# h3poteto/aws-global-accelerator-controller

Hardware: NVIDIA H100
Metric: objects reconciled/sec at 10^6 Service+Ingress; change-set bit-exact vs Go ref (higher is better)
Workload: dtype u8/u32 (bytes and indices)

## Files before the change

aws-global-accelerator-controller_b200/csrc/gar_common.h:

```cpp
#pragma once

#include <stdint.h>
#include <stddef.h>

#include "../../include/garecon.h"

#if defined(__CUDACC__)
#define GAR_HD __host__ __device__ __forceinline__
#define GAR_D __device__ __forceinline__
#else
#define GAR_HD inline
#define GAR_D inline
#endif

#if defined(__CUDA_ARCH__)
#define GAR_ANY(p) __any_sync(0xffffffffu, (p))
#else
bool gar_host_vote(bool p);
#define GAR_ANY(p) gar_host_vote((p))
#endif

typedef uint8_t u8;
typedef uint16_t u16;
typedef uint32_t u32;
// ... 238 lines not shown
  if (p.loaded) p.e = load_entry(ix.ent + p.c.pos);
  return p;
}
GAR_HD bool idx_next(const HashIdx &ix, PreCursor &p, IdxEntry *out) {
  while (p.c.pos < p.c.end) {
    if (!p.loaded) p.e = load_entry(ix.ent + p.c.pos);
    p.loaded = false;
    p.c.pos++;
    if (p.e.tag == p.c.tag) {
      *out = p.e;
      return true;
    }
  }
  return false;
}
```

aws-global-accelerator-controller_b200/csrc/gar_delta.h:

```cpp
#pragma once

#include <stddef.h>
#include <string.h>

#include <algorithm>
#include <string>
#include <unordered_map>
#include <unordered_set>
#include <vector>

#include "gar_pipeline.h"

enum DeltaCol {
  DC_KIND, DC_SPEC, DC_FLAGS, DC_NS, DC_NAME, DC_ICLS, DC_ANN_B, DC_LBI_B, DC_PORT_B, DC_ANN_KEY, DC_ANN_VAL, DC_LBI_HOST, DC_PORT_NUM,
  DC_PORT_PROTO, DC_N
};
enum ActualCol {
  AC_LB_REGION, AC_LB_NAME, AC_LB_DNS, AC_LB_ARN, AC_LB_STATE, AC_ACC_NAME, AC_ACC_DNS, AC_ACC_ENABLED, AC_ACC_TAG_B, AC_ACC_LIS_B, AC_TAG_KEY,
  AC_TAG_VAL, AC_LIS_PROTO, AC_LIS_PR_B, AC_LIS_EG_B, AC_PR_FROM, AC_EG_EP_B, AC_EP_ID, AC_ZONE_NAME, AC_ZONE_REC_B, AC_REC_NAME, AC_REC_TYPE,
  AC_REC_ALIAS, AC_REC_ALIAS_DNS, AC_REC_VAL_B, AC_VAL_VALUE, AC_N
};
enum ActualTable { AT_LB, AT_ACC, AT_TAG, AT_LIS, AT_PR, AT_EG, AT_EP, AT_ZONE, AT_REC, AT_VAL, AT_N };
enum DeltaScratch {
  DS_UP = 0, DS_KEY_KIND = DC_N, DS_KEY_REF, DS_KEY_SLAB, DS_COUNTS, DS_OFFS, DS_ROWS, DS_PAIRS, DS_SRC, DS_TOTALS,
  DS_A_UP, DS_A_SRC = DS_A_UP + AC_N, DS_A_DEL = DS_A_SRC + AT_N, DS_A_PAIRS = DS_A_DEL + AT_N, DS_A_ZTARGET = DS_A_PAIRS + AT_N, DS_A_ZREF,
  DS_A_ZSLAB, DS_A_FLAG, DS_A_COL, DS_N = DS_A_COL + 2 * AC_N
};

constexpr u32 SRC_UPSERT = 0x80000000u;

struct FDeltaResolve {
  DevTables T;
  HashIdx ix;
  const u8 *kind;
  const gar_str *key;
  const u8 *slab;
  u32 *counts;
  const u32 *offs;
  u32 *rows;
  GAR_HD void operator()(u32 k) const {
    const u32 kd = kind[k];
    const Str ks = mkstr(slab, key[k]);
    Cursor c = idx_open(ix, key_hash_kinded(kd, ks));
    IdxEntry e;
    u32 m = 0;
    while (idx_next(ix, c, &e))
      if (e.a0 == kd && streq(mkstr(T.o.slab, e.s0), ks)) {
        if (rows) rows[offs[k] + m] = e.row;
        m++;
      }
    if (!rows) counts[k] = m;
  }
};
struct FDeltaIdentity {
  u32 *src;
  GAR_HD void operator()(u32 i) const { src[i] = i; }
};
struct FDeltaScatter {
  const u32 *pairs;
  u32 *src;
  GAR_HD void operator()(u32 k) const { src[pairs[2 * k]] = pairs[2 * k + 1]; }
};
// ... 719 lines not shown
```

aws-global-accelerator-controller_b200/csrc/gar_pipeline.h:

```cpp
#pragma once

#include <stdio.h>
#include <stdlib.h>

#include <initializer_list>

#include "gar_rows.h"

#if defined(__CUDA_ARCH__)
#define GAR_ATOMIC_ADD(p, v) atomicAdd((p), (v))
#else
#define GAR_ATOMIC_ADD(p, v) (*(p) += (v))
#endif


enum Slot {
  S_DERIVED, S_OFLAGS, S_OKEY_HASH, S_STAGE_GA, S_STAGE_R53, S_ANN_R53, S_ANN_NAME, S_ANN_TAGS, S_ANN_LISTEN, S_DPORT_BEGIN, S_DPORTS,
  S_TOK_CODE, S_TOK_NAME, S_TOK_REGION,
  S_ACC_FLAGS, S_ACC_OWNER_KEY, S_ACC_OWNER, S_ACC_THOST, S_ACC_MANAGED, S_ACC_OWNER_HASH, S_ACC_THOST_HASH, S_REC_NAME_HASH, S_VAL_KEY_HASH,
  S_REC_ZONE, S_VAL_REC, S_VAL_CLS, S_VAL_KEY, S_VAL_ORPHAN, S_VAL_LINK, S_ACC_DIGEST,
  S_R53_MODE, S_R53_ACC, S_R53_ACC_DNS, S_PAIR_BEGIN, S_PAIR_OBJ, S_PAIR_HN, S_PAIR_CODE, S_PAIR_ZONE, S_PAIR_REC,
  S_IX_LB, S_IX_OWNER = S_IX_LB + 3, S_IX_THOST = S_IX_OWNER + 3, S_IX_ZONE = S_IX_THOST + 3, S_IX_VAL = S_IX_ZONE + 3,
  S_IX_ALIAS = S_IX_VAL + 3, S_IX_OBJ = S_IX_ALIAS + 3, S_IX_OVN = S_IX_OBJ + 3,
  S_SORT_KEYS = S_IX_OVN + 3, S_SORT_VALS, S_SORT_KEYS_ALT, S_SORT_VALS_ALT, S_SORT_TAGS,
  S_COUNTS, S_STATUS_GA, S_STATUS_R53, S_OPS, S_ERRFLAG, S_IX_EG, S_IX_EG_ENT, S_IX_EG_PAD,
  S_VAL_OBJ, S_ACC_OBJ, S_OBJ_CANON, S_OWN_BEGIN, S_OWN_FILL, S_OWN_ENT, S_OWN_MULTI,
  S_IXA_BEGIN, S_IXA_FILL, S_IXA_ENT, S_IXA_MULTI, S_OVN_FILL, S_OVN_MULTI, S_LB_HASH, S_REC_FLAGS, S_LBI_RES,
  S_NSLOTS
};


struct FClassify {
  DevTables T;
  Work W;
  u32 *derived_public;
  u8 *oflags;
  u32 *errflag;
  GAR_HD void operator()(u32 i) const {
    classify_object(T, W, i);
    W.obj_canon[i] = i;
    u32 dv = W.derived[i];
    if (dv & OBJ_KEY_BAD) GAR_ATOMIC_ADD(errflag, 1u);
// ... 130 lines not shown
    }
    W.dport_begin[i] = n;
  }
};
struct FJsonWrite {
  DevTables T;
  Work W;
  GAR_HD void operator()(u32 i) const {
    if (!(W.derived[i] & GAR_DV_PORTS_FROM_ANN)) return;
    if (W.dport_begin[i + 1] == W.dport_begin[i] || W.dport_begin[i + 1] > W.dport_cap) return;
    u32 stk[GAR_JSON_STACK_WORDS];
    json_listen_ports(mkstr(T.o.slab, W.ann_listen[i]), W.dports + W.dport_begin[i], stk);
  }
};

struct FLbHash {
  DevTables T;
  Work W;
  GAR_HD void operator()(u32 i) const {
    u64 h = key_hash_lb(mkstr(T.a.slab, T.a.lb_region[i]), mkstr(T.a.slab, T.a.lb_name[i]));
    W.lb_hash[i] = h;
    ix_count(W.hist[IX_LB], h);
  }
};
struct FRowLb {
  DevTables T;
  Work W;
  GAR_HD bool make(u32 i, u64 *h, IdxEntry *e) const {
    *h = W.lb_hash[i];
    e->a0 = T.a.lb_state[i];
    e->a1 = 0;
    e->s0 = T.a.lb_name[i];
    e->s1 = T.a.lb_region[i];
    return true;
  }
};
struct FRowOwner {
  DevTables T;
  Work W;
  GAR_HD bool make(u32 i, u64 *h, IdxEntry *e) const {
    u32 fl = W.acc_flags[i];
    *h = W.acc_owner_hash[i];
    e->a0 = fl;
    e->a1 = 0;
    e->s0 = W.acc_owner_key[i];
    e->s1 = 0;
    return (fl & ACC_MINE) && (fl & ACC_OWNER_KEYED) && i < W.acc_guest_from;
  }
// ... 57 lines not shown
struct FRowAlias {
  DevTables T;
  Work W;
  GAR_HD bool make(u32 r, u64 *h, IdxEntry *e) const {
    *h = key_hash_zoned_h(W.rec_zone[r], W.rec_name_hash[r]);
    e->a0 = W.rec_zone[r];
    e->a1 = T.a.rec_type[r];
    e->s0 = T.a.rec_name[r];
    e->s1 = T.a.rec_alias_dns[r];
    return T.a.rec_has_alias[r] != 0;
  }
};
struct FRowObj {
  DevTables T;
  Work W;
  GAR_HD bool make(u32 i, u64 *h, IdxEntry *e) const {
    gar_str ns = T.o.obj_ns[i];
    *h = W.okey_hash[i];
    e->a0 = T.o.obj_kind[i];
    e->a1 = 0;
    e->s0 = GAR_STR(GAR_STR_OFF(ns), GAR_STR_LEN(ns) + 1 + GAR_STR_LEN(T.o.obj_name[i]));
    e->s1 = 0;
    return !(W.derived[i] & OBJ_KEY_BAD);
  }
};
struct FRowOvn {
  DevTables T;
  Work W;
  GAR_HD bool make(u32 v, u64 *h, IdxEntry *e) const {
    u32 rec = W.val_rec[v];
    *h = key_hash_zoned_h(W.rec_zone[rec], W.rec_name_hash[rec]);
    e->a0 = rec;
    e->a1 = W.rec_zone[rec];
    e->s0 = T.a.rec_name[rec];
    e->s1 = T.a.val_value[v];
    return W.val_orphan[v] != 0;
  }
};

constexpr u32 IDX_SMALL_BUCKET = 48;
struct CanonHook {
  u32 *canon;
  const u8 *slab;
  u32 b0, b1;
  GAR_HD void operator()(u32 b, const IdxEntry *ent, u32 lo, u32 m) const {
    if (canon && b >= b0 && b < b1) canon_bucket(ent, lo, m, slab, canon);
  }
};
template <class RowF>
struct FIdxRows {
  RowF rowf;
  u32 *keys, *vals;
  IdxEntry *tmp;
  u32 *counts;
  u32 mask, nb;
  GAR_HD void operator()(u32 i) const {
    u64 h = 0;
    IdxEntry e;
    bool valid = rowf.make(i, &h, &e);
    u32 k = valid ? hash_bucket(h, mask) : nb;
    keys[i] = k;
    if (vals) vals[i] = i;
    if (valid) {
      e.tag = hash_tag(h);
      e.row = i;
      tmp[i] = e;
      GAR_ATOMIC_ADD(&counts[k], 1u);
    }
  }
};
struct FIdxPlace {
  const u32 *keys;
  u32 *cursor;
  const IdxEntry *tmp;
  IdxEntry *ent;
  u32 nb;
  GAR_HD void operator()(u32 i) const {
    u32 k = keys[i];
    if (k == nb) return;
#if defined(__CUDA_ARCH__)
    u32 pos = atomicAdd(&cursor[k], 1u);
#else
    u32 pos = cursor[k]++;
#endif
    ent[pos] = tmp[i];
  }
};
struct FIdxOrder {
  const u32 *begin;
  IdxEntry *ent;
  u32 *overflow;
  CanonHook canon;
  GAR_HD void operator()(u32 b) const {
    u32 lo = begin[b], m = begin[b + 1] - lo;
    if (m < 2) return;
    if (m > IDX_SMALL_BUCKET) {
      GAR_ATOMIC_ADD(overflow, 1u);
      return;
    }
    for (u32 k = 1; k < m; k++) {
      IdxEntry x = ent[lo + k];
      u32 j = k;
      while (j > 0 && ent[lo + j - 1].row > x.row) {
        ent[lo + j] = ent[lo + j - 1];
        j--;
      }
      if (j != k) ent[lo + j] = x;
    }
    canon(b, ent, lo, m);
  }
};
struct FIdxGather {
  const u32 *vals;
  const u32 *nvalid;
  const IdxEntry *tmp;
  IdxEntry *ent;
  GAR_HD void operator()(u32 p) const {
    if (p < *nvalid) ent[p] = tmp[vals[p]];
  }
};
struct FIdxCanon {
  const u32 *begin;
  const IdxEntry *ent;
  CanonHook canon;
  GAR_HD void operator()(u32 b) const {
    const u32 lo = begin[b], m = begin[b + 1] - lo;
    if (m >= 2) canon(b, ent, lo, m);
  }
};
template <class RowF>
struct FIdxPlaceDirect {
  RowF rowf;
  u32 *cursor;
  IdxEntry *ent;
  u32 mask;
  GAR_HD void operator()(u32 i) const {
    u64 h = 0;
    IdxEntry e;
    if (!rowf.make(i, &h, &e)) return;
    const u32 k = hash_bucket(h, mask);
#if defined(__CUDA_ARCH__)
    const u32 pos = atomicAdd(&cursor[k], 1u);
#else
    const u32 pos = cursor[k]++;
#endif
    e.tag = hash_tag(h);
    e.row = i;
    ent[pos] = e;
  }
};
struct FIdxMultiList {
  const u32 *begin;
  u32 *multi;
  GAR_HD void operator()(u32 b) const {
    const bool m = begin[b + 1] - begin[b] >= 2;
#if defined(__CUDA_ARCH__)
    const unsigned active = __activemask();
    const unsigned votes = __ballot_sync(active, m);
    if (!m) return;
    const unsigned lane = threadIdx.x & 31u;
    const int leader = __ffs(votes) - 1;
    u32 base = 0;
    if ((int)lane == leader) base = atomicAdd(multi, (u32)__popc(votes));
    base = __shfl_sync(votes, base, leader);
    multi[1 + base + __popc(votes & ((1u << lane) - 1u))] = b;
#else
    if (m) multi[1 + multi[0]++] = b;
#endif
  }
};
struct FIdxOrderMulti {
  const u32 *begin;
  IdxEntry *ent;
  const u32 *multi;
  u32 *overflow;
  CanonHook canon;
  GAR_HD void operator()(u32 t) const {
    const u32 b = multi[1 + t];
    const u32 lo = begin[b], m = begin[b + 1] - lo;
    if (m > IDX_SMALL_BUCKET) {
      GAR_ATOMIC_ADD(overflow, 1u);
      return;
    }
    for (u32 k = 1; k < m; k++) {
      IdxEntry x = ent[lo + k];
      u32 j = k;
      while (j > 0 && ent[lo + j - 1].row > x.row) {
        ent[lo + j] = ent[lo + j - 1];
        j--;
      }
      if (j != k) ent[lo + j] = x;
    }
    canon(b, ent, lo, m);
  }
};
enum FlagWord { FW_BAD_KEYS = 0, FW_IDX_OVERFLOW = 1, FW_NDPORTS = 2, FW_NPAIRS = 3, FW_SEC0 = 4 , FW_WORDS = 16 };
struct FGatherFinal {
  const u32 *src;
  u32 idx[5];
  const u32 *npairs;
  u32 *flags;
  GAR_HD void operator()(u32 k) const {
    if (k < 5) flags[FW_SEC0 + k] = src[idx[k]];
    else if (npairs) flags[FW_NPAIRS] = *npairs;
  }
};
struct FGather5 {
  const u32 *src;
// ... 331 lines not shown
}
inline int ilog2(u32 p) {
  int b = 0;
  while ((1u << b) < p) b++;
  return b;
}

template <class B>
struct Pipeline {
  B &be;
  DevTables T;
  Work W{};
  bool force_radix = false;
  explicit Pipeline(B &b, const DevTables &t) : be(b), T(t) {}

  template <class RowF>
  HashIdx build_index(int slot, u32 nrows, u32 load, RowF rowf, u32 *overflow, bool force_radix, CanonHook canon = {}) {
    u32 nb = next_pow2(nrows / load < 16 ? 16 : nrows / load);
    u32 *keys = (u32 *)be.ensure(S_SORT_KEYS, sizeof(u32) * (size_t)(nrows + 1));
    u32 *vals = (u32 *)be.ensure(S_SORT_VALS, sizeof(u32) * (size_t)(nrows + 1));
    IdxEntry *tmp = (IdxEntry *)be.ensure(S_SORT_TAGS, sizeof(IdxEntry) * (size_t)(nrows + 1));
    u32 *begin = (u32 *)be.ensure(slot + 0, sizeof(u32) * (size_t)(nb + 2));
    IdxEntry *ent = (IdxEntry *)be.ensure(slot + 1, sizeof(IdxEntry) * (size_t)(nrows + 1));
    be.fill32(begin, 0, nb + 2);
    if (nrows) be.for_each("idx_rows", nrows, FIdxRows<RowF>{rowf, keys, force_radix ? vals : nullptr, tmp, begin, nb - 1, nb});
    be.exclusive_scan(begin, nb + 2);
    if (nrows && !force_radix) {
      u32 *cursor = (u32 *)be.ensure(S_SORT_KEYS_ALT, sizeof(u32) * (size_t)(nb + 1));
      be.copy32(cursor, begin, nb);
      be.for_each("idx_place", nrows, FIdxPlace{keys, cursor, tmp, ent, nb});
      be.for_each("idx_order", nb, FIdxOrder{begin, ent, overflow, canon});
    } else if (nrows) {
      u32 *keys2 = (u32 *)be.ensure(S_SORT_KEYS_ALT, sizeof(u32) * (size_t)(nrows + 1));
      u32 *vals2 = (u32 *)be.ensure(S_SORT_VALS_ALT, sizeof(u32) * (size_t)(nrows + 1));
      be.sort_pairs(keys, vals, keys2, vals2, nrows, ilog2(nb) + 1);
      be.for_each("idx_gather", nrows, FIdxGather{vals, begin + nb, tmp, ent});
      if (canon.canon) be.for_each("idx_order", nb, FIdxCanon{begin, ent, canon});
    }
    return HashIdx{begin, ent, nb - 1};
  }

  bool prepared = false;
  u64 n_dports = 0;
  u32 *errflag = nullptr;

  u32 acc_guest_from = 0xFFFFFFFFu;
  u32 sharded = 0;
  bool orphan_sweep = true;
  bool allow_empty_cache = false;

  void alloc_obj_work() {
    const u32 n = T.o.n_objects, nlbi = T.o.n_lbi;
    W.derived = (u32 *)be.ensure(S_DERIVED, 4 * (size_t)(n + 1));
    W.okey_hash = (u64 *)be.ensure(S_OKEY_HASH, 8 * (size_t)(n + 1));
// ... 62 lines not shown
      be.fill32(big, 0, 1);
      be.fill32(huge, 0, 1);
      be.for_each_staged("prepare_records", nrec, FPrepareRecord{T, W, big, huge});
      if (nval > REC_INLINE_VALUES) be.for_each("prepare_records", BIG_BLOCKS * 256, FClassifyBigRecords{T, W, big, huge});
    }
  }
  struct IxPlan {
    u32 off[IX_N] = {}, nb[IX_N] = {}, rows[IX_N] = {};
    bool want[IX_N] = {};
    u32 total_nb = 0;
    u64 total_rows = 0;
  };
  IxPlan planA;
  u32 *ixa_begin = nullptr, *ixa_fill = nullptr, *ixa_multi = nullptr;
  IdxEntry *ixa_ent = nullptr;
  u32 ovn_nb = 0;
  void arm_group_a(u32 want_mask) {
    const u32 rows[IX_N] = {T.a.n_lbs, T.a.n_accels, T.a.n_accels, T.a.n_zones, T.a.n_values, T.a.n_records, T.o.n_objects, 0};
    const u32 load[IX_N] = {1, 1, 1, 1, 1, 2, 1, 8};
    planA = IxPlan{};
    for (int k = 0; k < IX_OVN; k++) {
      planA.want[k] = (want_mask >> k) & 1u;
      if (!planA.want[k]) continue;
      planA.rows[k] = rows[k];
      planA.nb[k] = next_pow2(rows[k] / load[k] < 16 ? 16 : rows[k] / load[k]);
      planA.off[k] = planA.total_nb;
      planA.total_nb += planA.nb[k];
      planA.total_rows += rows[k];
    }
    ixa_begin = (u32 *)be.ensure(S_IXA_BEGIN, 4 * (size_t)(planA.total_nb + 2));
    be.fill32(ixa_begin, 0, (size_t)planA.total_nb + 2);
    for (int k = 0; k < IX_OVN; k++)
      if (planA.want[k]) W.hist[k] = IxHist{ixa_begin + planA.off[k], planA.nb[k] - 1};
  }
  HashIdx group_a_index(int k) const { return HashIdx{ixa_begin + planA.off[k], ixa_ent, planA.nb[k] - 1}; }
  template <class RowF>
  FIdxPlaceDirect<RowF> placer(int k, RowF rowf) const {
    return FIdxPlaceDirect<RowF>{rowf, ixa_fill + planA.off[k], ixa_ent, planA.nb[k] - 1};
  }
  void finish_group_a() {
    u32 *overflow = errflag + FW_IDX_OVERFLOW;
    be.exclusive_scan(ixa_begin, planA.total_nb + 1);
    ixa_fill = (u32 *)be.ensure(S_IXA_FILL, 4 * (size_t)(planA.total_nb + 1));
    ixa_ent = (IdxEntry *)be.ensure(S_IXA_ENT, sizeof(IdxEntry) * (size_t)(planA.total_rows + 1));
    const u32 multi_cap = (u32)(planA.total_rows / 2 + 1);
    ixa_multi = (u32 *)be.ensure(S_IXA_MULTI, 4 * (size_t)(multi_cap + 2));
    be.copy32(ixa_fill, ixa_begin, (size_t)planA.total_nb + 1);
    be.fill32(ixa_multi, 0, 1);
    const IxPlan &P = planA;
    auto n = [&](int k) { return P.want[k] ? P.rows[k] : 0u; };
    be.for_each_multi("idx_place", {n(IX_LB), n(IX_THOST), n(IX_ZONE), n(IX_ALIAS), n(IX_OBJ), P.total_nb},
                      placer(IX_LB, FRowLb{T, W}), placer(IX_THOST, FRowThost{T, W}), placer(IX_ZONE, FRowZone{T}),
                      placer(IX_ALIAS, FRowAlias{T, W}), placer(IX_OBJ, FRowObj{T, W}), FIdxMultiList{ixa_begin, ixa_multi});
    const CanonHook canon = P.want[IX_OBJ] ? canon_hook(P.off[IX_OBJ], P.off[IX_OBJ] + P.nb[IX_OBJ]) : CanonHook{};
    be.for_each_dyn("idx_order", ixa_multi, multi_cap, FIdxOrderMulti{ixa_begin, ixa_ent, ixa_multi, overflow, canon});
    if (P.want[IX_LB]) W.ix_lb = group_a_index(IX_LB);
    if (P.want[IX_THOST]) W.ix_thost = group_a_index(IX_THOST);
    if (P.want[IX_ZONE]) W.ix_zone = group_a_index(IX_ZONE);
    if (P.want[IX_ALIAS]) W.ix_alias = group_a_index(IX_ALIAS);
    if (P.want[IX_OBJ]) W.ix_obj = group_a_index(IX_OBJ);
  }
  void resolve_owners(bool link_aliases) {
    const u32 n = T.o.n_objects, nacc = T.a.n_accels, nval = T.a.n_values, nseg = 2 * n;
    u32 *overflow = errflag + FW_IDX_OVERFLOW;
    W.own_begin = (u32 *)be.ensure(S_OWN_BEGIN, 4 * (size_t)(nseg + 2));
    be.fill32(W.own_begin, 0, (size_t)nseg + 1);
    u32 *ovn = nullptr;
    if (!force_radix) {
      ovn_nb = next_pow2(nval / 8 < 16 ? 16 : nval / 8);
      ovn = (u32 *)be.ensure(S_IX_OVN + 0, 4 * (size_t)(ovn_nb + 2));
      be.fill32(ovn, 0, (size_t)ovn_nb + 2);
      W.hist[IX_OVN] = IxHist{ovn, ovn_nb - 1};
    } else {
      W.hist[IX_OVN] = IxHist{nullptr, 0};
    }
// ... 2 lines not shown
    else be.for_each_multi("resolve_owners", {nval, nacc, nlbi}, FResolveValue{T, W}, FResolveAccel{T, W}, FLbiResolve{T, W});
    be.exclusive_scan(W.own_begin, nseg + 1);
    IdxEntry *own = (IdxEntry *)be.ensure(S_OWN_ENT, sizeof(IdxEntry) * ((size_t)nacc + nval + 1));
    if (!force_radix) {
      be.exclusive_scan(ovn, ovn_nb + 1);
      u32 *ovn_cursor = (u32 *)be.ensure(S_OVN_FILL, 4 * (size_t)(ovn_nb + 1));
      IdxEntry *ovn_ent = (IdxEntry *)be.ensure(S_IX_OVN + 1, sizeof(IdxEntry) * (size_t)(nval + 1));
      u32 *ovn_multi = (u32 *)be.ensure(S_OVN_MULTI, 4 * (size_t)(nval / 2 + 3));
      u32 *own_cursor = (u32 *)be.ensure(S_OWN_FILL, 4 * (size_t)(nseg + 1));
      const u32 own_multi_cap = (u32)(((u64)nacc + nval) / 2 + 1);
      u32 *own_multi = (u32 *)be.ensure(S_OWN_MULTI, 4 * (size_t)(own_multi_cap + 2));
      be.copy32(ovn_cursor, ovn, (size_t)ovn_nb + 1);
      be.copy32(own_cursor, W.own_begin, (size_t)nseg + 1);
      be.fill32(ovn_multi, 0, 1);
      be.fill32(own_multi, 0, 1);
      be.for_each_multi("idx_place", {nval, ovn_nb, nacc, nval, nseg}, FIdxPlaceDirect<FRowOvn>{FRowOvn{T, W}, ovn_cursor, ovn_ent, ovn_nb - 1},
                        FIdxMultiList{ovn, ovn_multi}, FOwnPlace{T, W, own_cursor, own, 0}, FOwnPlace{T, W, own_cursor, own, nacc},
                        FIdxMultiList{W.own_begin, own_multi});
      be.for_each_dyn("idx_order", ovn_multi, nval / 2 + 1, FIdxOrderMulti{ovn, ovn_ent, ovn_multi, overflow});
      be.for_each_dyn("idx_order", own_multi, own_multi_cap, FIdxOrderMulti{W.own_begin, own, own_multi, overflow});
      W.ix_ovn = HashIdx{ovn, ovn_ent, ovn_nb - 1};
    } else {
      const u32 nx = nacc + nval;
      u32 *keys = (u32 *)be.ensure(S_SORT_KEYS, 4 * (size_t)(nx + 1));
      u32 *vals = (u32 *)be.ensure(S_SORT_VALS, 4 * (size_t)(nx + 1));
      u32 *keys2 = (u32 *)be.ensure(S_SORT_KEYS_ALT, 4 * (size_t)(nx + 1));
      u32 *vals2 = (u32 *)be.ensure(S_SORT_VALS_ALT, 4 * (size_t)(nx + 1));
      if (nx) {
        be.for_each("own_keys", nx, FOwnKeys{T, W, keys, vals});
        be.sort_pairs(keys, vals, keys2, vals2, nx, ilog2(nseg + 1) + 1);
        be.for_each("own_gather", nx, FOwnGather{T, W, vals, W.own_begin + nseg, own});
// ... 438 lines not shown
```

aws-global-accelerator-controller_b200/csrc/gar_rows.h:

```cpp
#pragma once

#include "gar_common.h"
#include "gar_json.h"


struct DevTables {
  gar_objects o;
  gar_actual a;
  const u8 *cluster;
  u32 cluster_len;
};

enum {
  OBJ_HAS_NAME_ANN = 1u << 8,
  OBJ_HAS_TAGS_ANN = 1u << 9,
  OBJ_KEY_BAD = 1u << 10,
};

enum {
  ACC_MINE = 1u << 0,
  ACC_OWNER_KEYED = 1u << 1,
  ACC_OWNER_INGRESS = 1u << 2,
  ACC_OWNER_3PART = 1u << 3,
  ACC_HAS_MANAGED = 1u << 4, ACC_HAS_OWNER = 1u << 5, ACC_HAS_THOST = 1u << 6,
// ... 99 lines not shown
  u32 sharded;
  u32 *val_obj;
  u32 *acc_obj;
  u32 *obj_canon;
  u32 *own_begin;
  const IdxEntry *own;
  u8 *r53_mode;
  u32 *r53_acc;
  gar_str *r53_acc_dns;
  u32 *pair_begin;
  u32 *pair_obj;
  gar_str *pair_hn;
  u8 *pair_code;
  u32 *pair_zone;
  u32 *pair_rec;
  HashIdx ix_lb;
  HashIdx ix_owner;
  HashIdx ix_thost;
  HashIdx ix_zone;
  const u64 *zone_len_mask;
  HashIdx ix_val;
  HashIdx ix_alias;
  HashIdx ix_obj;
  HashIdx ix_ovn;
};

GAR_HD bool acc_in_owner_index(const Work &W, u32 a, u32 fl) { return (fl & ACC_MINE) && (fl & ACC_OWNER_KEYED) && a < W.acc_guest_from; }
GAR_HD bool acc_in_thost_index(const Work &W, u32 a, u32 fl) { return (fl & ACC_MINE) != 0 && (!W.sharded || a >= W.acc_guest_from); }


GAR_HD u64 key_hash_kinded(u32 kind, Str nsname) { return hmix(kind + 1, gar_hash(nsname)); }
GAR_HD u64 key_hash_lb(Str region, Str name) { return hmix(gar_hash(region), gar_hash(name)); }
GAR_HD u64 key_hash_zoned_h(u32 zone, u64 name_hash) { return hmix((u64)zone + 0x100, name_hash); }
GAR_HD u64 key_hash_zoned(u32 zone, Str name) { return key_hash_zoned_h(zone, gar_hash(name)); }
GAR_HD u64 key_hash_str(Str s) { return gar_hash(s); }

GAR_HD Str object_key(const DevTables &T, u32 i) {
  gar_str ns = T.o.obj_ns[i], nm = T.o.obj_name[i];
// ... 268 lines not shown
      key = GAR_STR(GAR_STR_OFF(ref) + ro + 8, rest.n - 8);
      if (count_slashes(substr(rest, 8, rest.n - 8)) == 1) cls |= VAL_OWNER_3PART;
    }
  }
  W.val_cls[v] = cls;
  W.val_key[v] = key;
  const u64 vkh = cls ? key_hash_kinded((cls & VAL_OWNER_INGRESS) ? 1u : 0u, substr(s, (u32)(GAR_STR_OFF(key) - GAR_STR_OFF(ref)), (u32)GAR_STR_LEN(key))) : 0;
  W.val_key_hash[v] = vkh;
  if (cls) ix_count(W.hist[IX_VAL], vkh);
}
GAR_HD void classify_value(const DevTables &T, const Work &W, u32 v) { classify_value_at(T, W, v, mkstr(T.a.slab, T.a.val_value[v])); }


template <class C>
GAR_HD u32 lb_walk(const DevTables &T, const Work &W, C &c, Str region, Str name, u32 *state) {
  IdxEntry e;
  while (idx_next(W.ix_lb, c, &e))
    if (streq(mkstr(T.a.slab, e.s0), name) && streq(mkstr(T.a.slab, e.s1), region)) {
      *state = e.a0;
      return e.row;
    }
  return GAR_NONE;
}
GAR_HD u32 find_lb(const DevTables &T, const Work &W, Str region, Str name, u32 *state) {
  Cursor c = idx_open(W.ix_lb, key_hash_lb(region, name));
  return lb_walk(T, W, c, region, name, state);
}

struct OwnRange {
  u32 pos, end;
};
GAR_HD OwnRange own_accs(const Work &W, u32 i) {
  const u32 s = 2 * W.obj_canon[i];
// ... 35 lines not shown
    }
    if (++n >= 2) break;
  }
  return n;
}
GAR_HD u32 find_by_hostname(const DevTables &T, const Work &W, Str hostname, u32 *first, gar_str *first_dns, u32 *second = nullptr) {
  Cursor c = idx_open(W.ix_thost, key_hash_str(hostname));
  return thost_walk(T, W, c, hostname, first, first_dns, second);
}

GAR_HD void lbi_resolve(const DevTables &T, const Work &W, u32 r) {
  if (W.tok_code[r] > GAR_TOK_NLB) return;
  const gar_actual &A = T.a;
  const Str host = mkstr(T.o.slab, T.o.lbi_hostname[r]);
  const Str region = mkstr(T.o.slab, W.tok_region[r]), name = mkstr(T.o.slab, W.tok_name[r]);
  PreCursor cl = idx_open_pre(W.ix_lb, key_hash_lb(region, name)), ch = idx_open_pre(W.ix_thost, key_hash_str(host));
  LbiRes res;
  u32 state = 0;
  const u32 lb = lb_walk(T, W, cl, region, name, &state);
  res.lb_dns = lb != GAR_NONE ? A.lb_dns[lb] : 0;
  res.lb_arn = lb != GAR_NONE ? A.lb_arn[lb] : 0;
  u32 acc = GAR_NONE;
  res.acc_dns = 0;
  const u32 nacc = thost_walk(T, W, ch, host, &acc, &res.acc_dns);
  res.acc = (nacc << 30) | (acc & LBI_ROW_MASK);
  res.lb = GAR_NONE;
  if (lb != GAR_NONE) {
    const u32 v = !streq(mkstr(A.slab, res.lb_dns), host) ? LBI_DNS_MISMATCH : state != GAR_LB_ACTIVE ? LBI_NOT_ACTIVE : LBI_OK;
    res.lb = (v << 30) | lb;
  }
  W.lbi_res[r] = res;
// ... 862 lines not shown
      } else if (code == PAIR_CREATE) {
        s.put(GAR_OP_HEAD(GAR_OP_R53_CREATE, GAR_CTRL_R53, kind), i, GAR_R53_SUB(0, k), W.pair_zone[p], acc, GAR_NONE);
        created = true;
      } else if (code == PAIR_UPSERT) {
        s.put(GAR_OP_HEAD(GAR_OP_R53_UPSERT_A, GAR_CTRL_R53, kind), i, GAR_R53_SUB(0, k), W.pair_zone[p], acc, W.pair_rec[p]);
      }
    }
    if (!stop) st = GAR_STATUS(GAR_ST_OK, 0, created ? GAR_EV_CREATED : 0);
  }
  return st;
}


GAR_HD u32 find_object(const DevTables &T, const Work &W, u32 kind, Str key, u64 key_hash) {
  Cursor c = idx_open(W.ix_obj, key_hash);
  IdxEntry e;
  while (idx_next(W.ix_obj, c, &e))
    if (e.a0 == kind && streq(mkstr(T.o.slab, e.s0), key)) return e.row;
  return GAR_NONE;
}
GAR_HD void canon_bucket(const IdxEntry *ent, u32 lo, u32 m, const u8 *oslab, u32 *canon) {
  for (u32 k = 1; k < m; k++) {
    const IdxEntry x = ent[lo + k];
    for (u32 j = 0; j < k; j++) {
      const IdxEntry y = ent[lo + j];
      if (y.tag == x.tag && y.a0 == x.a0 && streq(mkstr(oslab, y.s0), mkstr(oslab, x.s0))) {
        canon[x.row] = y.row;
        break;
      }
    }
  }
}

GAR_HD u32 ga_orphan(const DevTables &T, const Work &W, u32 acc, OpSink &s) {
  if (acc >= W.acc_guest_from) return 0;
  u32 fl = W.acc_flags[acc];
  if (!(fl & ACC_MINE) || !(fl & ACC_OWNER_3PART)) return 0;
  if (W.acc_obj[acc] != GAR_NONE) return 0;
  put_delete_chain(T, s, GAR_NONE, 0, acc);
  return 1;
}
// ... 23 lines not shown
  W.val_orphan[v] = orphan;
}

GAR_HD void value_joins(const DevTables &T, const Work &W, u32 v) {
  const u32 cls = W.val_cls[v];
  u32 row = GAR_NONE, o = GAR_NONE;
  gar_str dns = 0;
  if (cls != VAL_NOT_OWNER) {
    const u32 rec = W.val_rec[v], kind = (cls & VAL_OWNER_INGRESS) ? 1u : 0u;
    const gar_str kref = W.val_key[v];
    const u64 kh = W.val_key_hash[v];
    const u32 zone = W.rec_zone[rec];
    const gar_str nref = T.a.rec_name[rec];
    const u64 nh = W.rec_name_hash[rec];
    Cursor ca = idx_open(W.ix_alias, key_hash_zoned_h(zone, nh)), co = idx_open(W.ix_obj, kh);
    IdxEntry ea, eo;
    ea.tag = ~ca.tag;
    eo.tag = ~co.tag;
    if (ca.pos < ca.end) ea = load_entry(W.ix_alias.ent + ca.pos);
    if (co.pos < co.end) eo = load_entry(W.ix_obj.ent + co.pos);
    const Str name = mkstr(T.a.slab, nref), key = mkstr(T.a.slab, kref);
    while (ca.pos < ca.end) {
      if (ea.tag == ca.tag && ea.a0 == zone && ea.a1 == GAR_RR_A && streq(mkstr(T.a.slab, ea.s0), name)) {
        row = ea.row;
        dns = ea.s1;
        break;
      }
      if (++ca.pos < ca.end) ea = load_entry(W.ix_alias.ent + ca.pos);
    }
    while (co.pos < co.end) {
      if (eo.tag == co.tag && eo.a0 == kind && streq(mkstr(T.o.slab, eo.s0), key)) {
        o = eo.row;
        break;
      }
      if (++co.pos < co.end) eo = load_entry(W.ix_obj.ent + co.pos);
    }
    if (o != GAR_NONE) GAR_HIST_ADD(&W.own_begin[2 * o + 1]);
  }
  ValLink l;
  l.alias_row = row;
  l.pad = 0;
  l.alias_dns = dns;
  W.val_link[v] = l;
  W.val_obj[v] = o;
  const u8 orphan = (cls & VAL_OWNER_3PART) && o == GAR_NONE ? 1 : 0;
  if (orphan) {
// ... 79 lines not shown
      len--;
    }
    s.put(H(GAR_OP_EGB_UPDATE_STATUS), k, 0, GAR_NONE, GAR_NONE, GAR_NONE);
    return GAR_STATUS(GAR_ST_REQUEUE_1S, 0, 0);
  }
  if (!(flags & GAR_EGB_HAS_FINALIZERS)) {
    s.put(H(GAR_OP_EGB_ADD_FINALIZER), k, 0, GAR_NONE, GAR_NONE, GAR_NONE);
    return GAR_STATUS(GAR_ST_OK, 0, 0);
  }
  u32 jb = 0, nj = 0;
  u32 refkind = b.egb_ref_kind[k];
  if (refkind != GAR_EGB_REF_NONE) {
    u32 kind = refkind == GAR_EGB_REF_SERVICE ? GAR_KIND_SERVICE : GAR_KIND_INGRESS;
    Str key = mkstr(b.slab, b.egb_ref_key[k]);
    Cursor c = idx_open(W.ix_obj, key_hash_kinded(kind, key));
    IdxEntry e;
    u32 obj = GAR_NONE;
    while (idx_next(W.ix_obj, c, &e))
      if (e.a0 == kind && streq(mkstr(T.o.slab, e.s0), key)) {
        obj = e.row;
        break;
      }
    if (obj == GAR_NONE) return GAR_STATUS(GAR_ST_ERR_RETRY, GAR_D_REF_NOT_FOUND, 0);
    jb = T.o.obj_lbi_begin[obj];
    nj = T.o.obj_lbi_begin[obj + 1] - jb;
  }
  for (u32 j = 0; j < nj; j++) {
    u32 detail;
    if (egb_lb_of(T, W, jb + j, &detail) == GAR_NONE) return GAR_STATUS(GAR_ST_ERR_RETRY, detail, 0);
  }
  auto arn_of = [&](u32 j) {
    u32 d;
    return mkstr(A.slab, A.lb_arn[egb_lb_of(T, W, jb + j, &d)]);
  };
// ... 113 lines not shown
```

Baseline: 193.8 million.

## Inline short keys into 64-byte hash index entries for LB and object indices

Adds a KeyEntry layout that stores up to 48 bytes of key text inline in each index entry, falling back to slab references when keys are longer. The LB and object indices move to separate keyed entry arrays, and lookups compare against the inline bytes instead of chasing a pointer into the string slab. This is meant to remove the dependent random slab load on every tag hit during probing. In exchange, entries grow from 32 to 64 bytes, index build writes more data, bucket reordering moves larger records, and templating adds code complexity.

Result: no change. 195.0 million, median of 6 (+0.6%).

```diff
diff --git a/aws-global-accelerator-controller_b200/csrc/gar_common.h b/aws-global-accelerator-controller_b200/csrc/gar_common.h
--- a/aws-global-accelerator-controller_b200/csrc/gar_common.h
+++ b/aws-global-accelerator-controller_b200/csrc/gar_common.h
@@ -276,3 +276,114 @@
   }
   return false;
 }
+
+constexpr u32 KEY_INLINE = 48;
+constexpr u32 KEY_SPILLED = 0x80000000u;
+struct alignas(64) KeyEntry {
+  u32 tag, row, a0;
+  u32 len;
+  u64 key[KEY_INLINE / 8];
+};
+struct KeyIdx {
+  const u32 *begin;
+  const KeyEntry *ent;
+  u32 mask;
+};
+struct KeyHit {
+  u32 tag, row, a0, len;
+  const KeyEntry *p;
+};
+GAR_HD KeyHit load_entry(const KeyEntry *p) {
+  KeyHit e;
+#if defined(__CUDA_ARCH__)
+  const uint4 h = __ldg(reinterpret_cast<const uint4 *>(p));
+  e.tag = h.x;
+  e.row = h.y;
+  e.a0 = h.z;
+  e.len = h.w;
+#else
+  e.tag = p->tag;
+  e.row = p->row;
+  e.a0 = p->a0;
+  e.len = p->len;
+#endif
+  e.p = p;
+  return e;
+}
+GAR_HD Cursor idx_open(const KeyIdx &ix, u64 h) {
+  const u32 b = hash_bucket(h, ix.mask), base = ix.begin[0];
+  Cursor c;
+  c.pos = ix.begin[b] - base;
+  c.end = ix.begin[b + 1] - base;
+  c.tag = hash_tag(h);
+  return c;
+}
+GAR_HD bool idx_next(const KeyIdx &ix, Cursor &c, KeyHit *out) {
+  while (c.pos < c.end) {
+    KeyHit e = load_entry(ix.ent + c.pos++);
+    if (e.tag == c.tag) {
+      *out = e;
+      return true;
+    }
+  }
+  return false;
+}
+struct KeyPreCursor {
+  Cursor c;
+  KeyHit e;
+  bool loaded;
+};
+GAR_HD KeyPreCursor idx_open_pre(const KeyIdx &ix, u64 h) {
+  KeyPreCursor p;
+  p.c = idx_open(ix, h);
+  p.loaded = p.c.pos < p.c.end;
+  if (p.loaded) p.e = load_entry(ix.ent + p.c.pos);
+  return p;
+}
+GAR_HD bool idx_next(const KeyIdx &ix, KeyPreCursor &p, KeyHit *out) {
+  while (p.c.pos < p.c.end) {
+    if (!p.loaded) p.e = load_entry(ix.ent + p.c.pos);
+    p.loaded = false;
+    p.c.pos++;
+    if (p.e.tag == p.c.tag) {
+      *out = p.e;
+      return true;
+    }
+  }
+  return false;
+}
+GAR_HD Str key_part(const KeyHit &e, const u8 *slab, u32 k) {
+  if (e.len & KEY_SPILLED) return mkstr(slab, e.p->key[k]);
+  const u8 *b = reinterpret_cast<const u8 *>(e.p->key);
+  const u32 n0 = e.len & 0xFFFFu;
+  return k == 0 ? Str{b, n0} : Str{b + n0, (e.len >> 16) & 0x7FFFu};
+}
+GAR_HD void key_fill(KeyEntry *e, const u8 *slab, gar_str k0, gar_str k1) {
+  const Str s0 = mkstr(slab, k0), s1 = mkstr(slab, k1);
+  if (s0.n + s1.n > KEY_INLINE) {
+    e->len = KEY_SPILLED;
+    e->key[0] = k0;
+    e->key[1] = k1;
+    for (u32 i = 2; i < KEY_INLINE / 8; i++) e->key[i] = 0;
+    return;
+  }
+  e->len = s0.n | (s1.n << 16);
+  for (u32 i = 0; i < KEY_INLINE / 8; i++) {
+    const u32 at = 8 * i;
+    u64 w = at < s0.n ? load_word(s0, at) : 0;
+    if (at >= s0.n) {
+      if (at - s0.n < s1.n) w = load_word(s1, at - s0.n);
+    } else if (s0.n - at < 8 && s1.n) {
+      w |= load_word(s1, 0) << (8 * (s0.n - at));
+    }
+    e->key[i] = w;
+  }
+}
+GAR_HD bool key_eq(const KeyEntry &x, const KeyEntry &y, const u8 *slab) {
+  if (x.len != y.len) return false;
+  if (x.len & KEY_SPILLED)
+    return streq(mkstr(slab, x.key[0]), mkstr(slab, y.key[0])) && streq(mkstr(slab, x.key[1]), mkstr(slab, y.key[1]));
+  for (u32 i = 0; i < KEY_INLINE / 8; i++)
+    if (x.key[i] != y.key[i]) return false;
+  return true;
+}
diff --git a/aws-global-accelerator-controller_b200/csrc/gar_delta.h b/aws-global-accelerator-controller_b200/csrc/gar_delta.h
--- a/aws-global-accelerator-controller_b200/csrc/gar_delta.h
+++ b/aws-global-accelerator-controller_b200/csrc/gar_delta.h
@@ -31,7 +31,7 @@
 
 struct FDeltaResolve {
   DevTables T;
-  HashIdx ix;
+  KeyIdx ix;
   const u8 *kind;
   const gar_str *key;
   const u8 *slab;
@@ -42,10 +42,10 @@
     const u32 kd = kind[k];
     const Str ks = mkstr(slab, key[k]);
     Cursor c = idx_open(ix, key_hash_kinded(kd, ks));
-    IdxEntry e;
+    KeyHit e;
     u32 m = 0;
     while (idx_next(ix, c, &e))
-      if (e.a0 == kd && streq(mkstr(T.o.slab, e.s0), ks)) {
+      if (e.a0 == kd && streq(key_part(e, T.o.slab, 0), ks)) {
         if (rows) rows[offs[k] + m] = e.row;
         m++;
       }
diff --git a/aws-global-accelerator-controller_b200/csrc/gar_pipeline.h b/aws-global-accelerator-controller_b200/csrc/gar_pipeline.h
--- a/aws-global-accelerator-controller_b200/csrc/gar_pipeline.h
+++ b/aws-global-accelerator-controller_b200/csrc/gar_pipeline.h
@@ -25,7 +25,7 @@
   S_SORT_KEYS = S_IX_OVN + 3, S_SORT_VALS, S_SORT_KEYS_ALT, S_SORT_VALS_ALT, S_SORT_TAGS,
   S_COUNTS, S_STATUS_GA, S_STATUS_R53, S_OPS, S_ERRFLAG, S_IX_EG, S_IX_EG_ENT, S_IX_EG_PAD,
   S_VAL_OBJ, S_ACC_OBJ, S_OBJ_CANON, S_OWN_BEGIN, S_OWN_FILL, S_OWN_ENT, S_OWN_MULTI,
-  S_IXA_BEGIN, S_IXA_FILL, S_IXA_ENT, S_IXA_MULTI, S_OVN_FILL, S_OVN_MULTI, S_LB_HASH, S_REC_FLAGS, S_LBI_RES,
+  S_IXA_BEGIN, S_IXA_FILL, S_IXA_ENT, S_IXA_LB_ENT, S_IXA_OBJ_ENT, S_IXA_MULTI, S_OVN_FILL, S_OVN_MULTI, S_LB_HASH, S_REC_FLAGS, S_LBI_RES,
   S_NSLOTS
 };
 
@@ -186,6 +186,18 @@
   }
 };
 
+template <class R, class E>
+E entry_of(bool (R::*)(u32, u64 *, E *) const);
+template <class RowF>
+using EntryOf = decltype(entry_of(&RowF::make));
+template <class E>
+struct IdxOf {
+  typedef HashIdx type;
+};
+template <>
+struct IdxOf<KeyEntry> {
+  typedef KeyIdx type;
+};
 struct FLbHash {
   DevTables T;
   Work W;
@@ -198,12 +210,10 @@
 struct FRowLb {
   DevTables T;
   Work W;
-  GAR_HD bool make(u32 i, u64 *h, IdxEntry *e) const {
+  GAR_HD bool make(u32 i, u64 *h, KeyEntry *e) const {
     *h = W.lb_hash[i];
     e->a0 = T.a.lb_state[i];
-    e->a1 = 0;
-    e->s0 = T.a.lb_name[i];
-    e->s1 = T.a.lb_region[i];
+    key_fill(e, T.a.slab, T.a.lb_name[i], T.a.lb_region[i]);
     return true;
   }
 };
@@ -291,14 +301,13 @@
 struct FRowObj {
   DevTables T;
   Work W;
-  GAR_HD bool make(u32 i, u64 *h, IdxEntry *e) const {
+  GAR_HD bool make(u32 i, u64 *h, KeyEntry *e) const {
+    const bool valid = !(W.derived[i] & OBJ_KEY_BAD);
     gar_str ns = T.o.obj_ns[i];
     *h = W.okey_hash[i];
     e->a0 = T.o.obj_kind[i];
-    e->a1 = 0;
-    e->s0 = GAR_STR(GAR_STR_OFF(ns), GAR_STR_LEN(ns) + 1 + GAR_STR_LEN(T.o.obj_name[i]));
-    e->s1 = 0;
-    return !(W.derived[i] & OBJ_KEY_BAD);
+    if (valid) key_fill(e, T.o.slab, GAR_STR(GAR_STR_OFF(ns), GAR_STR_LEN(ns) + 1 + GAR_STR_LEN(T.o.obj_name[i])), 0);
+    return valid;
   }
 };
 struct FRowOvn {
@@ -320,20 +329,33 @@
   u32 *canon;
   const u8 *slab;
   u32 b0, b1;
-  GAR_HD void operator()(u32 b, const IdxEntry *ent, u32 lo, u32 m) const {
+  GAR_HD void operator()(u32, const IdxEntry *, u32, u32) const {}
+  GAR_HD void operator()(u32 b, const KeyEntry *ent, u32 lo, u32 m) const {
     if (canon && b >= b0 && b < b1) canon_bucket(ent, lo, m, slab, canon);
   }
 };
+template <class E>
+GAR_HD void order_bucket(E *ent, u32 lo, u32 m) {
+  for (u32 k = 1; k < m; k++) {
+    E x = ent[lo + k];
+    u32 j = k;
+    while (j > 0 && ent[lo + j - 1].row > x.row) {
+      ent[lo + j] = ent[lo + j - 1];
+      j--;
+    }
+    if (j != k) ent[lo + j] = x;
+  }
+}
 template <class RowF>
 struct FIdxRows {
   RowF rowf;
   u32 *keys, *vals;
-  IdxEntry *tmp;
+  EntryOf<RowF> *tmp;
   u32 *counts;
   u32 mask, nb;
   GAR_HD void operator()(u32 i) const {
     u64 h = 0;
-    IdxEntry e;
+    EntryOf<RowF> e;
     bool valid = rowf.make(i, &h, &e);
     u32 k = valid ? hash_bucket(h, mask) : nb;
     keys[i] = k;
@@ -346,11 +368,12 @@
     }
   }
 };
+template <class E>
 struct FIdxPlace {
   const u32 *keys;
   u32 *cursor;
-  const IdxEntry *tmp;
-  IdxEntry *ent;
+  const E *tmp;
+  E *ent;
   u32 nb;
   GAR_HD void operator()(u32 i) const {
     u32 k = keys[i];
@@ -363,9 +386,10 @@
     ent[pos] = tmp[i];
   }
 };
+template <class E>
 struct FIdxOrder {
   const u32 *begin;
-  IdxEntry *ent;
+  E *ent;
   u32 *overflow;
   CanonHook canon;
   GAR_HD void operator()(u32 b) const {
@@ -375,30 +399,24 @@
       GAR_ATOMIC_ADD(overflow, 1u);
       return;
     }
-    for (u32 k = 1; k < m; k++) {
-      IdxEntry x = ent[lo + k];
-      u32 j = k;
-      while (j > 0 && ent[lo + j - 1].row > x.row) {
-        ent[lo + j] = ent[lo + j - 1];
-        j--;
-      }
-      if (j != k) ent[lo + j] = x;
-    }
+    order_bucket(ent, lo, m);
     canon(b, ent, lo, m);
   }
 };
+template <class E>
 struct FIdxGather {
   const u32 *vals;
   const u32 *nvalid;
-  const IdxEntry *tmp;
-  IdxEntry *ent;
+  const E *tmp;
+  E *ent;
   GAR_HD void operator()(u32 p) const {
     if (p < *nvalid) ent[p] = tmp[vals[p]];
   }
 };
+template <class E>
 struct FIdxCanon {
   const u32 *begin;
-  const IdxEntry *ent;
+  const E *ent;
   CanonHook canon;
   GAR_HD void operator()(u32 b) const {
     const u32 lo = begin[b], m = begin[b + 1] - lo;
@@ -409,11 +427,12 @@
 struct FIdxPlaceDirect {
   RowF rowf;
   u32 *cursor;
-  IdxEntry *ent;
+  EntryOf<RowF> *ent;
+  const u32 *base;
   u32 mask;
   GAR_HD void operator()(u32 i) const {
     u64 h = 0;
-    IdxEntry e;
+    EntryOf<RowF> e;
     if (!rowf.make(i, &h, &e)) return;
     const u32 k = hash_bucket(h, mask);
 #if defined(__CUDA_ARCH__)
@@ -423,7 +442,7 @@
 #endif
     e.tag = hash_tag(h);
     e.row = i;
-    ent[pos] = e;
+    ent[base ? pos - base[0] : pos] = e;
   }
 };
 struct FIdxMultiList {
@@ -446,12 +465,17 @@
 #endif
   }
 };
+struct KeySlice {
+  KeyEntry *ent;
+  u32 b0, b1;
+};
 struct FIdxOrderMulti {
   const u32 *begin;
   IdxEntry *ent;
   const u32 *multi;
   u32 *overflow;
   CanonHook canon;
+  KeySlice keyed[2];
   GAR_HD void operator()(u32 t) const {
     const u32 b = multi[1 + t];
     const u32 lo = begin[b], m = begin[b + 1] - lo;
@@ -459,16 +483,14 @@
       GAR_ATOMIC_ADD(overflow, 1u);
       return;
     }
-    for (u32 k = 1; k < m; k++) {
-      IdxEntry x = ent[lo + k];
-      u32 j = k;
-      while (j > 0 && ent[lo + j - 1].row > x.row) {
-        ent[lo + j] = ent[lo + j - 1];
-        j--;
+    for (const KeySlice &k : keyed)
+      if (b >= k.b0 && b < k.b1) {
+        const u32 klo = lo - begin[k.b0];
+        order_bucket(k.ent, klo, m);
+        canon(b, k.ent, klo, m);
+        return;
       }
-      if (j != k) ent[lo + j] = x;
-    }
-    canon(b, ent, lo, m);
+    order_bucket(ent, lo, m);
   }
 };
 enum FlagWord { FW_BAD_KEYS = 0, FW_IDX_OVERFLOW = 1, FW_NDPORTS = 2, FW_NPAIRS = 3, FW_SEC0 = 4 , FW_WORDS = 16 };
@@ -830,30 +852,30 @@
   bool force_radix = false;
   explicit Pipeline(B &b, const DevTables &t) : be(b), T(t) {}
 
-  template <class RowF>
-  HashIdx build_index(int slot, u32 nrows, u32 load, RowF rowf, u32 *overflow, bool force_radix, CanonHook canon = {}) {
+  template <class RowF, class E = EntryOf<RowF>>
+  typename IdxOf<E>::type build_index(int slot, u32 nrows, u32 load, RowF rowf, u32 *overflow, bool force_radix, CanonHook canon = {}) {
     u32 nb = next_pow2(nrows / load < 16 ? 16 : nrows / load);
     u32 *keys = (u32 *)be.ensure(S_SORT_KEYS, sizeof(u32) * (size_t)(nrows + 1));
     u32 *vals = (u32 *)be.ensure(S_SORT_VALS, sizeof(u32) * (size_t)(nrows + 1));
-    IdxEntry *tmp = (IdxEntry *)be.ensure(S_SORT_TAGS, sizeof(IdxEntry) * (size_t)(nrows + 1));
+    E *tmp = (E *)be.ensure(S_SORT_TAGS, sizeof(E) * (size_t)(nrows + 1));
     u32 *begin = (u32 *)be.ensure(slot + 0, sizeof(u32) * (size_t)(nb + 2));
-    IdxEntry *ent = (IdxEntry *)be.ensure(slot + 1, sizeof(IdxEntry) * (size_t)(nrows + 1));
+    E *ent = (E *)be.ensure(slot + 1, sizeof(E) * (size_t)(nrows + 1));
     be.fill32(begin, 0, nb + 2);
     if (nrows) be.for_each("idx_rows", nrows, FIdxRows<RowF>{rowf, keys, force_radix ? vals : nullptr, tmp, begin, nb - 1, nb});
     be.exclusive_scan(begin, nb + 2);
     if (nrows && !force_radix) {
       u32 *cursor = (u32 *)be.ensure(S_SORT_KEYS_ALT, sizeof(u32) * (size_t)(nb + 1));
       be.copy32(cursor, begin, nb);
-      be.for_each("idx_place", nrows, FIdxPlace{keys, cursor, tmp, ent, nb});
-      be.for_each("idx_order", nb, FIdxOrder{begin, ent, overflow, canon});
+      be.for_each("idx_place", nrows, FIdxPlace<E>{keys, cursor, tmp, ent, nb});
+      be.for_each("idx_order", nb, FIdxOrder<E>{begin, ent, overflow, canon});
     } else if (nrows) {
       u32 *keys2 = (u32 *)be.ensure(S_SORT_KEYS_ALT, sizeof(u32) * (size_t)(nrows + 1));
       u32 *vals2 = (u32 *)be.ensure(S_SORT_VALS_ALT, sizeof(u32) * (size_t)(nrows + 1));
       be.sort_pairs(keys, vals, keys2, vals2, nrows, ilog2(nb) + 1);
-      be.for_each("idx_gather", nrows, FIdxGather{vals, begin + nb, tmp, ent});
-      if (canon.canon) be.for_each("idx_order", nb, FIdxCanon{begin, ent, canon});
-    }
-    return HashIdx{begin, ent, nb - 1};
+      be.for_each("idx_gather", nrows, FIdxGather<E>{vals, begin + nb, tmp, ent});
+      if (canon.canon) be.for_each("idx_order", nb, FIdxCanon<E>{begin, ent, canon});
+    }
+    return typename IdxOf<E>::type{begin, ent, nb - 1};
   }
 
   bool prepared = false;
@@ -946,6 +968,7 @@
   IxPlan planA;
   u32 *ixa_begin = nullptr, *ixa_fill = nullptr, *ixa_multi = nullptr;
   IdxEntry *ixa_ent = nullptr;
+  KeyEntry *ixa_lb_ent = nullptr, *ixa_obj_ent = nullptr;
   u32 ovn_nb = 0;
   void arm_group_a(u32 want_mask) {
     const u32 rows[IX_N] = {T.a.n_lbs, T.a.n_accels, T.a.n_accels, T.a.n_zones, T.a.n_values, T.a.n_records, T.o.n_objects, 0};
@@ -966,15 +989,25 @@
       if (planA.want[k]) W.hist[k] = IxHist{ixa_begin + planA.off[k], planA.nb[k] - 1};
   }
   HashIdx group_a_index(int k) const { return HashIdx{ixa_begin + planA.off[k], ixa_ent, planA.nb[k] - 1}; }
+  KeyIdx group_a_keyed(int k, const KeyEntry *ent) const { return KeyIdx{ixa_begin + planA.off[k], ent, planA.nb[k] - 1}; }
   template <class RowF>
   FIdxPlaceDirect<RowF> placer(int k, RowF rowf) const {
-    return FIdxPlaceDirect<RowF>{rowf, ixa_fill + planA.off[k], ixa_ent, planA.nb[k] - 1};
+    return FIdxPlaceDirect<RowF>{rowf, ixa_fill + planA.off[k], ixa_ent, nullptr, planA.nb[k] - 1};
+  }
+  template <class RowF>
+  FIdxPlaceDirect<RowF> placer(int k, RowF rowf, KeyEntry *ent) const {
+    return FIdxPlaceDirect<RowF>{rowf, ixa_fill + planA.off[k], ent, ixa_begin + planA.off[k], planA.nb[k] - 1};
+  }
+  KeySlice key_slice(int k, KeyEntry *ent) const {
+    return planA.want[k] ? KeySlice{ent, planA.off[k], planA.off[k] + planA.nb[k]} : KeySlice{nullptr, 0, 0};
   }
   void finish_group_a() {
     u32 *overflow = errflag + FW_IDX_OVERFLOW;
     be.exclusive_scan(ixa_begin, planA.total_nb + 1);
     ixa_fill = (u32 *)be.ensure(S_IXA_FILL, 4 * (size_t)(planA.total_nb + 1));
     ixa_ent = (IdxEntry *)be.ensure(S_IXA_ENT, sizeof(IdxEntry) * (size_t)(planA.total_rows + 1));
+    ixa_lb_ent = (KeyEntry *)be.ensure(S_IXA_LB_ENT, sizeof(KeyEntry) * ((size_t)planA.rows[IX_LB] + 1));
+    ixa_obj_ent = (KeyEntry *)be.ensure(S_IXA_OBJ_ENT, sizeof(KeyEntry) * ((size_t)planA.rows[IX_OBJ] + 1));
     const u32 multi_cap = (u32)(planA.total_rows / 2 + 1);
     ixa_multi = (u32 *)be.ensure(S_IXA_MULTI, 4 * (size_t)(multi_cap + 2));
     be.copy32(ixa_fill, ixa_begin, (size_t)planA.total_nb + 1);
@@ -982,15 +1015,16 @@
     const IxPlan &P = planA;
     auto n = [&](int k) { return P.want[k] ? P.rows[k] : 0u; };
     be.for_each_multi("idx_place", {n(IX_LB), n(IX_THOST), n(IX_ZONE), n(IX_ALIAS), n(IX_OBJ), P.total_nb},
-                      placer(IX_LB, FRowLb{T, W}), placer(IX_THOST, FRowThost{T, W}), placer(IX_ZONE, FRowZone{T}),
-                      placer(IX_ALIAS, FRowAlias{T, W}), placer(IX_OBJ, FRowObj{T, W}), FIdxMultiList{ixa_begin, ixa_multi});
+                      placer(IX_LB, FRowLb{T, W}, ixa_lb_ent), placer(IX_THOST, FRowThost{T, W}), placer(IX_ZONE, FRowZone{T}),
+                      placer(IX_ALIAS, FRowAlias{T, W}), placer(IX_OBJ, FRowObj{T, W}, ixa_obj_ent), FIdxMultiList{ixa_begin, ixa_multi});
     const CanonHook canon = P.want[IX_OBJ] ? canon_hook(P.off[IX_OBJ], P.off[IX_OBJ] + P.nb[IX_OBJ]) : CanonHook{};
-    be.for_each_dyn("idx_order", ixa_multi, multi_cap, FIdxOrderMulti{ixa_begin, ixa_ent, ixa_multi, overflow, canon});
-    if (P.want[IX_LB]) W.ix_lb = group_a_index(IX_LB);
+    be.for_each_dyn("idx_order", ixa_multi, multi_cap,
+                    FIdxOrderMulti{ixa_begin, ixa_ent, ixa_multi, overflow, canon, {key_slice(IX_LB, ixa_lb_ent), key_slice(IX_OBJ, ixa_obj_ent)}});
+    if (P.want[IX_LB]) W.ix_lb = group_a_keyed(IX_LB, ixa_lb_ent);
     if (P.want[IX_THOST]) W.ix_thost = group_a_index(IX_THOST);
     if (P.want[IX_ZONE]) W.ix_zone = group_a_index(IX_ZONE);
     if (P.want[IX_ALIAS]) W.ix_alias = group_a_index(IX_ALIAS);
-    if (P.want[IX_OBJ]) W.ix_obj = group_a_index(IX_OBJ);
+    if (P.want[IX_OBJ]) W.ix_obj = group_a_keyed(IX_OBJ, ixa_obj_ent);
   }
   void resolve_owners(bool link_aliases) {
     const u32 n = T.o.n_objects, nacc = T.a.n_accels, nval = T.a.n_values, nseg = 2 * n;
@@ -1023,7 +1057,7 @@
       be.copy32(own_cursor, W.own_begin, (size_t)nseg + 1);
       be.fill32(ovn_multi, 0, 1);
       be.fill32(own_multi, 0, 1);
-      be.for_each_multi("idx_place", {nval, ovn_nb, nacc, nval, nseg}, FIdxPlaceDirect<FRowOvn>{FRowOvn{T, W}, ovn_cursor, ovn_ent, ovn_nb - 1},
+      be.for_each_multi("idx_place", {nval, ovn_nb, nacc, nval, nseg}, FIdxPlaceDirect<FRowOvn>{FRowOvn{T, W}, ovn_cursor, ovn_ent, nullptr, ovn_nb - 1},
                         FIdxMultiList{ovn, ovn_multi}, FOwnPlace{T, W, own_cursor, own, 0}, FOwnPlace{T, W, own_cursor, own, nacc},
                         FIdxMultiList{W.own_begin, own_multi});
       be.for_each_dyn("idx_order", ovn_multi, nval / 2 + 1, FIdxOrderMulti{ovn, ovn_ent, ovn_multi, overflow});
diff --git a/aws-global-accelerator-controller_b200/csrc/gar_rows.h b/aws-global-accelerator-controller_b200/csrc/gar_rows.h
--- a/aws-global-accelerator-controller_b200/csrc/gar_rows.h
+++ b/aws-global-accelerator-controller_b200/csrc/gar_rows.h
@@ -137,14 +137,14 @@
   u8 *pair_code;
   u32 *pair_zone;
   u32 *pair_rec;
-  HashIdx ix_lb;
+  KeyIdx ix_lb;
   HashIdx ix_owner;
   HashIdx ix_thost;
   HashIdx ix_zone;
   const u64 *zone_len_mask;
   HashIdx ix_val;
   HashIdx ix_alias;
-  HashIdx ix_obj;
+  KeyIdx ix_obj;
   HashIdx ix_ovn;
 };
 
@@ -443,9 +443,9 @@
 
 template <class C>
 GAR_HD u32 lb_walk(const DevTables &T, const Work &W, C &c, Str region, Str name, u32 *state) {
-  IdxEntry e;
+  KeyHit e;
   while (idx_next(W.ix_lb, c, &e))
-    if (streq(mkstr(T.a.slab, e.s0), name) && streq(mkstr(T.a.slab, e.s1), region)) {
+    if (streq(key_part(e, T.a.slab, 0), name) && streq(key_part(e, T.a.slab, 1), region)) {
       *state = e.a0;
       return e.row;
     }
@@ -511,7 +511,8 @@
   const gar_actual &A = T.a;
   const Str host = mkstr(T.o.slab, T.o.lbi_hostname[r]);
   const Str region = mkstr(T.o.slab, W.tok_region[r]), name = mkstr(T.o.slab, W.tok_name[r]);
-  PreCursor cl = idx_open_pre(W.ix_lb, key_hash_lb(region, name)), ch = idx_open_pre(W.ix_thost, key_hash_str(host));
+  KeyPreCursor cl = idx_open_pre(W.ix_lb, key_hash_lb(region, name));
+  PreCursor ch = idx_open_pre(W.ix_thost, key_hash_str(host));
   LbiRes res;
   u32 state = 0;
   const u32 lb = lb_walk(T, W, cl, region, name, &state);
@@ -1404,17 +1405,17 @@
 
 GAR_HD u32 find_object(const DevTables &T, const Work &W, u32 kind, Str key, u64 key_hash) {
   Cursor c = idx_open(W.ix_obj, key_hash);
-  IdxEntry e;
+  KeyHit e;
   while (idx_next(W.ix_obj, c, &e))
-    if (e.a0 == kind && streq(mkstr(T.o.slab, e.s0), key)) return e.row;
+    if (e.a0 == kind && streq(key_part(e, T.o.slab, 0), key)) return e.row;
   return GAR_NONE;
 }
-GAR_HD void canon_bucket(const IdxEntry *ent, u32 lo, u32 m, const u8 *oslab, u32 *canon) {
+GAR_HD void canon_bucket(const KeyEntry *ent, u32 lo, u32 m, const u8 *oslab, u32 *canon) {
   for (u32 k = 1; k < m; k++) {
-    const IdxEntry x = ent[lo + k];
+    const KeyEntry &x = ent[lo + k];
     for (u32 j = 0; j < k; j++) {
-      const IdxEntry y = ent[lo + j];
-      if (y.tag == x.tag && y.a0 == x.a0 && streq(mkstr(oslab, y.s0), mkstr(oslab, x.s0))) {
+      const KeyEntry &y = ent[lo + j];
+      if (y.tag == x.tag && y.a0 == x.a0 && key_eq(y, x, oslab)) {
         canon[x.row] = y.row;
         break;
       }
@@ -1468,7 +1469,8 @@
     const gar_str nref = T.a.rec_name[rec];
     const u64 nh = W.rec_name_hash[rec];
     Cursor ca = idx_open(W.ix_alias, key_hash_zoned_h(zone, nh)), co = idx_open(W.ix_obj, kh);
-    IdxEntry ea, eo;
+    IdxEntry ea;
+    KeyHit eo;
     ea.tag = ~ca.tag;
     eo.tag = ~co.tag;
     if (ca.pos < ca.end) ea = load_entry(W.ix_alias.ent + ca.pos);
@@ -1483,7 +1485,7 @@
       if (++ca.pos < ca.end) ea = load_entry(W.ix_alias.ent + ca.pos);
     }
     while (co.pos < co.end) {
-      if (eo.tag == co.tag && eo.a0 == kind && streq(mkstr(T.o.slab, eo.s0), key)) {
+      if (eo.tag == co.tag && eo.a0 == kind && streq(key_part(eo, T.o.slab, 0), key)) {
         o = eo.row;
         break;
       }
@@ -1593,10 +1595,10 @@
     u32 kind = refkind == GAR_EGB_REF_SERVICE ? GAR_KIND_SERVICE : GAR_KIND_INGRESS;
     Str key = mkstr(b.slab, b.egb_ref_key[k]);
     Cursor c = idx_open(W.ix_obj, key_hash_kinded(kind, key));
-    IdxEntry e;
+    KeyHit e;
     u32 obj = GAR_NONE;
     while (idx_next(W.ix_obj, c, &e))
-      if (e.a0 == kind && streq(mkstr(T.o.slab, e.s0), key)) {
+      if (e.a0 == kind && streq(key_part(e, T.o.slab, 0), key)) {
         obj = e.row;
         break;
       }
```
